# skokec/DAU-ConvNet

Measured on AMD Instinct MI355X. Metric: DAU fwd+bwd GSamples/s (N*H*W/s), higher is better.
Workload: dtype f32

## Files before the change

### dau-convnet_amd/csrc/dau_conv_api.hip

```cpp
#include <cmath>
#include <cstdarg>
#include <cstdio>
#include <algorithm>
#include <atomic>
#include <cstring>
#include <memory>
#include <mutex>
#include <new>
#include <string>
#include <utility>
#include <vector>

#include "dau_common.hpp"
#include "dau_tiled.hpp"

using namespace dau;

namespace {

thread_local std::string g_last_error;

int fail(int code, const char* fmt, ...) {
    char buf[512];
    va_list ap;
// ... 641 lines not shown
    if (!plan || !info) return fail(DAU_INVALID_ARGUMENT, "null argument");
    info->offset_bucket = plan->bucket;
    info->blur_support = plan->blur_k;
    info->algo_forward = plan->algo_fwd;
    info->algo_backward = plan->algo_bwd;
    info->drop_last_col = plan->drop_col;
    info->drop_last_row = plan->drop_row;
    const BucketSet& top = plan->top();
    const bool* s0 = plan->sets[0].has;
    const bool tiled_fwd = plan->algo_fwd == DAU_ALGO_TILED;
    info->gather_patch = tiled_fwd ? top.tiled[kFwd].tiles_x * top.tiled[kFwd].tile_w : 0;
    info->gather_stack = tiled_fwd ? top.tiled[kFwd].stack : 0;
    info->dot_windows = plan->algo_bwd == DAU_ALGO_TILED ? top.tiled_dot.windows : 0;
    info->gather_windows = tiled_fwd ? top.tiled[kFwd].windows : 0;
    info->bucket_sets = plan->dynamic ? plan->nsets : 1;
    const bool dense_reachable = s0[kBf16R4] && (plan->nsets == 1 || plan->dynamic);
    info->gather_dense_bf16 = dense_reachable ? (s0[kWgradR4] ? 2 : 1) : 0;
    info->batch_slab_gather = top.slab_gather;
    info->batch_slab_dot = top.slab_dot;
    info->dot_region = top.has[kTiledDot] ? top.tiled_dot.region_cols * 100 + top.tiled_dot.region_rows : 0;
    info->gather_fblock = tiled_fwd ? top.tiled[kFwd].fblock : 0;
    info->gather_variant = tiled_fwd ? top.tiled[kFwd].variant : -1;
    info->dense_bf16_radius3 = dense_reachable && plan->dynamic && s0[kBf16R3] ? (s0[kWgradR3] ? 2 : 1) : 0;
    info->gather_dense_split = 0;
    if (plan->dynamic && tiled_fwd)
        for (int m = kSplit2; m <= kSplit4; ++m)
            if (s0[m]) info->gather_dense_split |= 1 << kRadius[m];
    if (plan->sets[0].ring) info->gather_dense_split |= 1 << 5;
    if (plan->dynamic && tiled_fwd && s0[kLine4]) info->gather_dense_split |= 1 << 6;
    if (plan->dynamic && tiled_fwd && s0[kLine8]) info->gather_dense_split |= 1 << 7;
    return DAU_OK;
}

int dau_conv_workspace_bytes(const dau_conv_plan* plan, int pass, size_t* bytes_out) {
    if (!plan || !bytes_out) return fail(DAU_INVALID_ARGUMENT, "null argument");
    if (pass == DAU_PASS_FORWARD) *bytes_out = carve_forward(plan, nullptr).bytes;
    else if (pass == DAU_PASS_BACKWARD) *bytes_out = carve_backward(plan, nullptr).bytes;
    else if (pass == DAU_PASS_EPILOGUE_BACKWARD)
        *bytes_out = epilogue_grad_workspace_bytes(plan->sh.N, plan->sh.F, plan->sh.H, plan->sh.W, plan->act(), plan->d.flags & DAU_FLAG_IO_NHWC);
    else return fail(DAU_INVALID_ARGUMENT, "pass must be DAU_PASS_FORWARD, DAU_PASS_BACKWARD or DAU_PASS_EPILOGUE_BACKWARD");
    return DAU_OK;
}

namespace {
int forward_pass(const dau_conv_plan* p, void* stream, const float* x, const float* w, const float* mu1,
                 const float* mu2, const float* sigma, float* y, void* workspace, size_t workspace_bytes, const Epilogue& epi) {
    if (!p || !x || !w || !mu1 || !mu2 || !sigma || !y || !workspace) return fail(DAU_INVALID_ARGUMENT, "null argument");
    FwdWs ws = carve_forward(p, workspace);
    if (workspace_bytes < ws.bytes)
        return fail(DAU_INVALID_ARGUMENT, "workspace too small: %zu < %zu", workspace_bytes, ws.bytes);
    hipStream_t st = static_cast<hipStream_t>(stream);
    if (int rc = ensure_attrs(p)) return rc;
    DAU_HIP(hipMemsetAsync(ws.status, 0, sizeof(Status), st));
    launch_synth_filters(st, sigma, p->blur_k, p->d.flags, ws.filters);
    launch_prepare_units(st, w, mu1, mu2, p->sh, p->d.number_units_ignore, p->d.flags, p->bucket, false, ws.table, ws.status,
                         p->host_status, -1, p->sets[0].has[kLine4] ? ws.status : nullptr);
    run_gather_sum(p, st, kFwd, x, y, ws.filters, ws.table, ws.status, ws.gather, epi);
    DAU_HIP(hipPeekAtLastError());
    return DAU_OK;
}
}

int dau_conv_forward(const dau_conv_plan* p, void* stream, const float* x, const float* w, const float* mu1,
                     const float* mu2, const float* sigma, float* y, void* workspace, size_t workspace_bytes) {
    return forward_pass(p, stream, x, w, mu1, mu2, sigma, y, workspace, workspace_bytes, Epilogue{});
}
// ... 248 lines not shown
```

### dau-convnet_amd/csrc/dau_tiled.hpp

```cpp
#pragma once
#include "dau_common.hpp"

namespace dau {

struct TiledConfig {
    int N, Cin, Cout, G, H, W;
    int R;
    int blur_k;
    int NP;
    int windows;
    int stack;
    int patches;
    int rows, pitch;
    int tiles_x, tiles_y;
    int tile_w;
    int fblock;
    int variant;
    int debug;
    int act;
    int nhwc;
    int in_relu;
};

bool tiled_gather_configure(int N, int Cin, int Cout, int G, int H, int W, int R, int blur_k, int act, TiledConfig* cfg);
// ... 82 lines not shown
    int debug;
    int nhwc;
    int in_relu;
};

bool tiled_dot_configure(const Shape& sh, int R, int blur_k, int act, int ignore, TiledDotConfig* cfg);
size_t tiled_dot_workspace_bytes(const TiledDotConfig& cfg);
void tiled_dot_prepare(hipStream_t st, const TiledDotConfig& cfg, const float* x, const float* dy,
                       const float* filters, const UnitRef* table_bare, int drop_col, int drop_row, void* workspace,
                       const Guard& guard);
void tiled_dot_run(hipStream_t st, const TiledDotConfig& cfg, float* r4, void* workspace, const Guard& guard, bool accumulate);
void tiled_dot_init(const TiledDotConfig& cfg);

void launch_blur4_pack(hipStream_t st, const float* x, const float* filters, int N, int C, int cstride, int H, int W, int Hp,
                       int Wp, int blur_k, int act, float* xk, const Guard& guard, unsigned* kmax = nullptr, bool nhwc = false,
                       bool in_relu = false);
void blur4_pack_init(int blur_k, bool kmax = false, bool nhwc = false);
bool blur4_pack_fits(int blur_k, int Hp, int Wp);

void launch_dot_reduce(hipStream_t st, const void* partial, int partial_f32, long n, int G, int F, int g_split, int slabs0,
                       int slabs1, int zero_from, bool accumulate, float* r4, const Guard& guard);

struct SplitDotConfig {
    Shape sh;
    int blur_k;
    int RW;
    int act;
    int e_limbs;
    int nhwc;
    int in_relu;
};
bool split_dot_configure(const Shape& sh, int blur_k, int act, SplitDotConfig* cfg);
size_t split_dot_workspace_bytes(const SplitDotConfig& cfg);
void split_dot_init(const SplitDotConfig& cfg);
void split_dot_prepare(hipStream_t st, const SplitDotConfig& cfg, const float* x, const float* dy, const float* filters,
                       int drop_col, int drop_row, void* workspace, const Guard& guard);
void split_dot_run(hipStream_t st, const SplitDotConfig& cfg, const UnitRef* table, float* r4, void* workspace, const Guard& guard);

struct WgradConfig {
    Shape sh;
    int blur_k;
    int SB, FB, NC;
    int HsT, WsT, WT, nseg;
    int splits;
    int Hp, Wp;
    bool fused;
};
#define DAU_DECLARE_DENSE_WGRAD(NS)                                                                                            \
    namespace NS {                                                                                                            \
    bool dense_wgrad_configure(const Shape& sh, int blur_k, bool bf16, WgradConfig* cfg);                                     \
    size_t dense_wgrad_workspace_bytes(const WgradConfig& cfg);                                                               \
    void dense_wgrad_init(const WgradConfig& cfg);                                                                            \
    void dense_wgrad_run(hipStream_t st, const WgradConfig& cfg, const float* x, const float* dy, const float* filters,       \
                         const UnitRef* table, int drop_col, int drop_row, float* r4, void* workspace, const Guard& guard, int nk); \
    }
DAU_DECLARE_DENSE_WGRAD(r4)
DAU_DECLARE_DENSE_WGRAD(r3)

size_t epilogue_grad_workspace_bytes(long N, int F, int H, int W, int act, bool nhwc);
bool epilogue_grad_run(hipStream_t st, long N, int F, int H, int W, int act, bool nhwc, const float* dy, const float* y, bool relu,
                       float* dz, float* dbias, void* workspace);

}
```

### dau-convnet_amd/csrc/k_split_dot.hip

```cpp
#include <algorithm>
#include <cfloat>

#include "dau_tiled.hpp"

namespace dau {

typedef _Float16 h8 __attribute__((ext_vector_type(8)));
typedef float f4s __attribute__((ext_vector_type(4)));

namespace {

constexpr int kSdWaves = 8;
constexpr int kSdAS = 2;
constexpr int kSdGT = 4;
constexpr int kSdSB = kSdWaves * kSdAS;
constexpr int kSdFB = 16;
constexpr int kSdR = 4;
constexpr int kSdRH = 4;
constexpr int kSdFlushItems = 16;
constexpr unsigned kVmcnt0 = 0x0F70, kVmcnt8 = 0x0F78;

inline size_t rup(size_t v, size_t a = 256) { return (v + a - 1) / a * a; }

struct SdGeom {
    int Hq, Wq, rq, cq, XTr, XTc, EYs, EXs, octs, nfb, nsb, ngb, items, chunks, per, NP;
};

SdGeom sd_geom(const SplitDotConfig& c) {
    const Shape& s = c.sh;
    SdGeom g{};
    g.Hq = (s.H + 1 + kSdRH - 1) / kSdRH * kSdRH;
    g.Wq = (s.W + 1 + c.RW - 1) / c.RW * c.RW;
    g.rq = g.Hq / kSdRH; g.cq = g.Wq / c.RW;
    g.XTr = g.Hq + 1; g.XTc = g.Wq + 1;
    g.EYs = g.Hq + 2 * kSdR; g.EXs = g.Wq + 2 * kSdR;
    g.octs = (s.N + 7) / 8;
    g.NP = (s.N + 1) / 2;
    g.nfb = (s.F + kSdFB - 1) / kSdFB;
    g.nsb = (s.S + kSdSB - 1) / kSdSB;
    g.ngb = (s.G + kSdGT - 1) / kSdGT;
    g.items = g.octs * g.rq * g.cq;
    const int per_chunk = g.nfb * g.nsb * g.ngb;
    int chunks = (1024 + per_chunk - 1) / per_chunk;
    chunks = std::max(1, std::min(chunks, g.items));
    g.per = (g.items + chunks - 1) / chunks;
    g.chunks = (g.items + g.per - 1) / g.per;
    return g;
}

struct SdLayout { size_t maxes_off, xk_off, xs_off, es_off, partial_off, total; };

SdLayout sd_layout(const SplitDotConfig& c, const SdGeom& g) {
    const Shape& s = c.sh;
    SdLayout l{};
    size_t off = 0;
    l.maxes_off = off; off += rup((size_t)(s.S * kNumK + s.F) * 4);
    l.xk_off = off; off += rup((size_t)g.NP * s.S * s.H * s.W * 32);
    l.xs_off = off; off += rup((size_t)g.octs * s.S * kNumK * g.XTr * g.XTc * 32 + 32);
    l.es_off = off; off += rup((size_t)g.octs * g.nfb * g.EYs * g.EXs * 256 * c.e_limbs);
    l.partial_off = off; off += rup((size_t)g.chunks * kNumK * s.S * s.G * s.F * 4);
    l.total = off;
    return l;
}

__device__ __forceinline__ int sd_shift(unsigned maxbits) {
    if (maxbits == 0u) return 0;
// ... 533 lines not shown
        const float sc = f < F ? ldexpf(1.0f, sd_shift(emax[f])) : 0.0f;
        float v[8];
#pragma unroll
        for (int n = 0; n < 8; ++n) {
            const int img = oct * 8 + n;
            const bool ok = in && img < N;
            v[n] = mask_act(load_act(dy, ok ? nhwc_index(img, f, y, x, F, H, W) : 0, act), ok);
        }
        h8 hi, lo;
#pragma unroll
        for (int n = 0; n < 8; ++n) {
            if constexpr (LIMBS == 2) {
                _Float16 h, l;
                split_limbs(v[n] * sc, &h, &l);
                hi[n] = h; lo[n] = l;
            } else {
                hi[n] = (_Float16)(v[n] * sc);
            }
        }
        dst[lx * (kSdFB * LIMBS) + fl] = hi;
        if constexpr (LIMBS == 2) dst[lx * (kSdFB * LIMBS) + kSdFB + fl] = lo;
    }
}

struct SdArgs {
    const h8* xs;
    const char* es;
    const unsigned* xmax;
    const unsigned* emax;
    const UnitRef* table;
    float* partial;
    int S, F, G;
    int nfb, nsb, ngb, per, items, rq, cq, XTr, XTc, EYs, EXs;
    Guard guard;
};

__device__ __forceinline__ void sd_glds16(const char* src, unsigned dst) {
    unsigned keep;
    asm volatile("s_mov_b32 %0, m0\n\ts_mov_b32 m0, %2\n\ts_nop 0\n\tglobal_load_lds_dwordx4 %1, off\n\ts_mov_b32 m0, %0"
                 : "=&s"(keep) : "v"(src), "s"(dst) : "memory");
}

#ifndef DAU_SD_STEP_LOADS
__device__ __forceinline__ h8 sd_next_col(h8 cur, h8 nxt, int dx) {
    typedef int i4s __attribute__((ext_vector_type(4)));
    const i4s c = __builtin_bit_cast(i4s, cur), n = __builtin_bit_cast(i4s, nxt);
    i4s r;
#pragma unroll
    for (int d = 0; d < 4; ++d)
        r[d] = __builtin_amdgcn_update_dpp(0, dx ? c[d] : n[d], 0xB1 , 0xF, 0xF, true);
    return __builtin_bit_cast(h8, r);
}
#endif

template <int RW, int EL>
__device__ __forceinline__ void sd_dot_body(const SdArgs& a) {
    extern __shared__ __attribute__((aligned(16))) char lds[];
    if (!guard_pass(a.guard)) return;
    constexpr int WL = RW + 2 * kSdR, WR = kSdRH + 2 * kSdR;
    constexpr int kRing = WR + kSdRH;
    constexpr int PB = EL * 256;
    constexpr unsigned RB = WL * PB;
    constexpr int kRowPieces = (RB + 1023) / 1024;
    static_assert((kRing & (kRing - 1)) == 0, "ring slot = (origin + row) & (kRing - 1)");
    static_assert(RW % 2 == 0, "A fragment sets by the parity of the K step / of the pair of K steps");
#ifdef DAU_SD_STEP_LOADS
// ... 13 lines not shown
    const int fl = lane & 15, j = lane >> 4;
    const int f = fb * kSdFB + fl;
    const bool f_ok = f < a.F;
    const unsigned lds0 = (unsigned)(uintptr_t)(__attribute__((address_space(3))) char*)lds;
    const int m = lane & 15, ak = m >> 2, ady = (m >> 1) & 1, adx = m & 1;
    const size_t xplane = (size_t)a.XTr * a.XTc;
    unsigned aoff[kSdAS];
    int sidx[kSdAS];
    bool s_ok[kSdAS];
    unsigned uw[kSdAS][kSdGT];
    f4s wb[kSdAS][kSdGT];
    float run[kSdAS][kSdGT];
#pragma unroll
    for (int i = 0; i < kSdAS; ++i) {
        const int s = sb * kSdSB + wave * kSdAS + i;
        s_ok[i] = s < a.S;
        sidx[i] = s_ok[i] ? s : a.S - 1;
        aoff[i] = (unsigned)((((size_t)sidx[i] * kNumK + ak) * xplane + (size_t)(j + ady) * a.XTc + adx) * 2);
#pragma unroll
        for (int gg = 0; gg < kSdGT; ++gg) {
            const int g = gb * kSdGT + gg;
            UnitRef u{0, 0, 0.0f, 0.0f, 0.0f, 0.0f};
            if (s_ok[i] && g < a.G && f_ok) u = a.table[((size_t)sidx[i] * a.G + g) * a.F + f];
            uw[i][gg] = (unsigned)(j - u.oy + kSdR) | (unsigned)((kSdR - u.ox) * PB + fl * 16) << 4;
            wb[i][gg] = f4s{u.w00, u.w01, u.w10, u.w11};
            run[i][gg] = 0.0f;
        }
    }
    int shx[kSdAS];
    const int she = f_ok ? sd_shift(a.emax[f]) : 0;
#pragma unroll
    for (int i = 0; i < kSdAS; ++i) shx[i] = sd_shift(a.xmax[sidx[i] * kNumK + j]);
    auto flush = [&]() {
#pragma unroll
        for (int i = 0; i < kSdAS; ++i) {
#pragma unroll
            for (int gg = 0; gg < kSdGT; ++gg) {
                const int g = gb * kSdGT + gg;
                if (s_ok[i] && g < a.G && f_ok) {
                    const float v = ldexpf(ldexpf(run[i][gg], -shx[i]), -she);
                    float* dst = a.partial + ((((size_t)chunk * kNumK + j) * a.S + sidx[i]) * a.G + g) * a.F + f;
                    __hip_atomic_fetch_add(dst, v, __ATOMIC_RELAXED, __HIP_MEMORY_SCOPE_AGENT);
                }
                run[i][gg] = 0.0f;
            }
        }
    };
    const int per_oct = a.rq * a.cq;
    auto item_off = [&](int item) {
        const int oct = item / per_oct, reg = item - oct * per_oct, rx = reg / a.rq, ry = reg - rx * a.rq;
        return ((size_t)oct * a.S * kNumK * xplane + (size_t)(ry * kSdRH) * a.XTc + (size_t)rx * RW) * 2;
    };
    auto fill = [&](int oct, int ry, int rx, int w0, int nrows, int origin) {
#ifndef DAU_SD_DIAG_NOFILL
        const char* src = a.es + ((((size_t)oct * a.nfb + fb) * a.EYs + (size_t)(ry * kSdRH + w0)) * a.EXs + (size_t)rx * RW) * PB;
        for (int u = wave_u; u < nrows * kRowPieces; u += kSdWaves) {
            const int rr = u / kRowPieces, pc = u - rr * kRowPieces;
            const unsigned within = pc * 1024 + lane * 16;
            const unsigned slot = (unsigned)(origin + w0 + rr) & (kRing - 1);
            if (within < RB) sd_glds16(src + (size_t)rr * a.EXs * PB + within, lds0 + slot * RB + pc * 1024);
        }
#endif
    };
    h8 ahi[2][kSdAS], alo[2][kSdAS];
    if (it0 < it1) {
#pragma unroll
        for (int p = 0; p < 2; ++p)
#pragma unroll
            for (int i = 0; i < kSdAS; ++i) {
                const h8* ap = a.xs + item_off(it0) + (size_t)p * kSdAStride + aoff[i];
                ahi[p][i] = ap[0]; alo[p][i] = ap[1];
            }
    }
    int since_flush = 0;
    int origin = 0;
    for (int it = it0; it < it1; ++it) {
        const int oct = it / per_oct, reg = it - oct * per_oct, rx = reg / a.rq, ry = reg - rx * a.rq;
        __builtin_amdgcn_s_waitcnt(kVmcnt8);
        __syncthreads();
        if (it > it0 && ry > 0) {
            origin = (origin + kSdRH) & (kRing - 1);
        } else {
            origin = 0;
            fill(oct, ry, rx, 0, WR, 0);
            __builtin_amdgcn_s_waitcnt(kVmcnt0);
            __syncthreads();
        }
        if (it + 1 < it1 && ry + 1 < a.rq) fill(oct, ry, rx, WR, kSdRH, origin);
        int base[kSdAS][kSdGT];
#pragma unroll
        for (int i = 0; i < kSdAS; ++i)
#pragma unroll
            for (int gg = 0; gg < kSdGT; ++gg)
                base[i][gg] = (int)((((unsigned)origin + (uw[i][gg] & 15u)) & (kRing - 1)) * RB + (uw[i][gg] >> 4));
#ifdef DAU_SD_DIAG_AFIXED
        const size_t ioff = item_off(it0), ioff_next = ioff;
#else
        const size_t ioff = item_off(it);
        const size_t ioff_next = item_off(it + 1 < it1 ? it + 1 : it);
#endif
        f4s part[kSdAS][kSdGT];
#pragma unroll
        for (int i = 0; i < kSdAS; ++i)
#pragma unroll
            for (int gg = 0; gg < kSdGT; ++gg) part[i][gg] = f4s{0.0f, 0.0f, 0.0f, 0.0f};
#ifdef DAU_SD_DIAG_NOA
#define SD_LOAD_A(P, i, an)
#else
#define SD_LOAD_A(P, i, an) { const h8* ap = a.xs + (an) + aoff[i]; ahi[P][i] = ap[0]; alo[P][i] = ap[1]; }
#endif
#define SD_READ_B(i, bh, bl)                                                                                    \
    _Pragma("unroll") for (int gg = 0; gg < kSdGT; ++gg) {                                                      \
        const char* bp = lds + base[i][gg] + k * PB;                                                            \
        bh[gg] = *reinterpret_cast<const h8*>(bp);                                                              \
        if constexpr (EL == 2) bl[gg] = *reinterpret_cast<const h8*>(bp + 256);                                 \
    }
#define SD_GROUP(i, AH, AL, bh, bl, AFTER)                                                                      \
    __builtin_amdgcn_sched_barrier(0);                                                                          \
    _Pragma("unroll") for (int gg = 0; gg < kSdGT; ++gg) {                                                      \
        part[i][gg] = __builtin_amdgcn_mfma_f32_16x16x32_f16(AH, bh[gg], part[i][gg], 0, 0, 0);                 \
        part[i][gg] = __builtin_amdgcn_mfma_f32_16x16x32_f16(AL, bh[gg], part[i][gg], 0, 0, 0);                 \
        if constexpr (EL == 2) part[i][gg] = __builtin_amdgcn_mfma_f32_16x16x32_f16(AH, bl[gg], part[i][gg], 0, 0, 0); \
    }                                                                                                           \
    AFTER                                                                                                       \
    __builtin_amdgcn_sched_barrier(0);
#define SD_STEP(kk, AH, AL, AFTER0, AFTER1)                                                                     \
    {                                                                                                           \
        const int k = (kk);                                                                                     \
        h8 b0h[kSdGT], b0l[kSdGT], b1h[kSdGT], b1l[kSdGT];                                                      \
        SD_READ_B(0, b0h, b0l)                                                                                  \
        SD_READ_B(1, b1h, b1l)                                                                                  \
        SD_GROUP(0, AH[0], AL[0], b0h, b0l, AFTER0)                                                             \
        SD_GROUP(1, AH[1], AL[1], b1h, b1l, AFTER1)                                                             \
    }
        static_assert(kSdAS == 2, "two groups per K step");
#ifdef DAU_SD_STEP_LOADS
#define SD_STEP1(P, kk)                                                                                         \
    {                                                                                                           \
        const size_t an = (kk) + 2 < RW ? ioff + (size_t)((kk) + 2) * 2 : ioff_next + (size_t)((kk) + 2 - RW) * 2; \
        (void)an;                                                                                               \
        SD_STEP(kk, ahi[P], alo[P], SD_LOAD_A(P, 0, an), SD_LOAD_A(P, 1, an))                                   \
    }
#pragma unroll 1
        for (int k2 = 0; k2 < RW; k2 += 2) {
            SD_STEP1(0, k2)
            SD_STEP1(1, k2 + 1)
        }
#undef SD_STEP1
#else
        h8 aqh[kSdAS], aql[kSdAS];
#define SD_NEXT_COL(P, i)                                                                                       \
    aqh[i] = sd_next_col(ahi[P][i], ahi[1 - (P)][i], adx);                                                      \
    aql[i] = sd_next_col(alo[P][i], alo[1 - (P)][i], adx);
#define SD_PAIR(P, rr)                                                                                          \
    {                                                                                                           \
        const size_t an = ioff + (size_t)((rr) + 2) * 4;                                                        \
        (void)an;                                                                                               \
        SD_STEP(2 * (rr), ahi[P], alo[P], SD_NEXT_COL(P, 0) SD_LOAD_A(P, 0, an), SD_NEXT_COL(P, 1) SD_LOAD_A(P, 1, an)) \
        SD_STEP(2 * (rr) + 1, aqh, aql, , )                                                                     \
    }
#define SD_PAIR_LAST(P, rr)                                                                                     \
    {                                                                                                           \
        SD_STEP(2 * (rr), ahi[P], alo[P], SD_NEXT_COL(P, 0) SD_LOAD_A(0, 0, ioff_next), SD_NEXT_COL(P, 1) SD_LOAD_A(0, 1, ioff_next)) \
        SD_STEP(2 * (rr) + 1, aqh, aql, SD_LOAD_A(1, 0, ioff_next + 4), SD_LOAD_A(1, 1, ioff_next + 4))         \
    }
        constexpr int kPairs = RW / 2, kLoopPairs = (kPairs - 1) / 2 * 2;
#pragma unroll 1
        for (int r2 = 0; r2 < kLoopPairs; r2 += 2) {
            SD_PAIR(0, r2)
            SD_PAIR(1, r2 + 1)
        }
        if constexpr (kPairs - kLoopPairs == 2) {
            SD_PAIR(0, kPairs - 2)
            SD_PAIR_LAST(1, kPairs - 1)
        } else {
            SD_PAIR_LAST(0, kPairs - 1)
        }
#undef SD_NEXT_COL
#undef SD_PAIR
#undef SD_PAIR_LAST
#endif
#undef SD_READ_B
#undef SD_GROUP
#undef SD_LOAD_A
#undef SD_STEP
#pragma unroll
        for (int i = 0; i < kSdAS; ++i)
#pragma unroll
            for (int gg = 0; gg < kSdGT; ++gg) {
                const int g = gb * kSdGT + gg;
                const bool ok = s_ok[i] && g < a.G && f_ok;
                const f4s p = part[i][gg], w = wb[i][gg];
                float v = w[0] * p[0];
                v = fmaf(w[1], p[1], v);
                v = fmaf(w[2], p[2], v);
                v = fmaf(w[3], p[3], v);
                run[i][gg] += ok ? v : 0.0f;
            }
        if (++since_flush == kSdFlushItems) { flush(); since_flush = 0; }
    }
    asm volatile("s_waitcnt vmcnt(0)" ::: "memory");
    if (since_flush) flush();
}

template <int RW>
__global__ void __launch_bounds__(kSdWaves * 64) __attribute__((amdgpu_waves_per_eu(2, 2))) split_gather_dot_kernel(const SdArgs a) {
    sd_dot_body<RW, 2>(a);
}

template <int RW>
__global__ void __launch_bounds__(kSdWaves * 64) __attribute__((amdgpu_waves_per_eu(2, 2))) sd_e1_dot_kernel(const SdArgs a) {
    sd_dot_body<RW, 1>(a);
}

template <int RW, int EL>
void launch_sd(hipStream_t st, const SdArgs* a, int grid) {
    auto kern = [] { if constexpr (EL == 2) return split_gather_dot_kernel<RW>; else return sd_e1_dot_kernel<RW>; }();
    const size_t lds = (size_t)(2 * kSdRH + 2 * kSdR) * (RW + 2 * kSdR) * 256 * EL;
    if (!a) { (void)hipFuncSetAttribute(reinterpret_cast<const void*>(kern), hipFuncAttributeMaxDynamicSharedMemorySize, 160 * 1024); return; }
    hipLaunchKernelGGL(kern, dim3(grid), dim3(kSdWaves * 64), lds, st, *a);
}
bool sd_walks(const SplitDotConfig& c) {
#if defined(DAU_SD_XK_COPY) || defined(DAU_SD_STAGE_REF)
    return false;
#else
    const SdGeom g = sd_geom(c);
    const long nct = (g.XTc + kXwCols - 1) / kXwCols;
    return !c.nhwc && (c.blur_k == 5 || c.blur_k == 7 || c.blur_k == 9) && (long)g.octs * c.sh.S * nct < (1L << 31);
#endif
}
template <int K, bool STORE>
void launch_xk_walk(hipStream_t st, const XkWalkArgs& a, int grid) {
// ... 19 lines not shown
        else launch_sd<12, 1>(st, a, grid);
    } else {
        if (RW == 10) launch_sd<10, 2>(st, a, grid);
        else launch_sd<12, 2>(st, a, grid);
    }
}

}

bool split_dot_configure(const Shape& sh, int blur_k, int act, SplitDotConfig* cfg) {
    int best = 0;
    long best_cost = 1L << 40;
    for (int rw = 12; rw >= 10; rw -= 2) {
        const long wq = (sh.W + 1 + rw - 1) / rw * rw;
        const long cost = wq * (rw + 2) * (60 / rw);
        if (cost < best_cost) { best_cost = cost; best = rw; }
    }
    if ((size_t)(2 * kSdRH + 2 * kSdR) * (best + 2 * kSdR) * 512 > 160 * 1024) return false;
    if (!blur4_pack_fits(blur_k, sh.H, sh.W)) return false;
    SplitDotConfig c{};
    c.sh = sh; c.blur_k = blur_k; c.RW = best; c.act = act;
#ifdef DAU_SD_BF16_E2
    c.e_limbs = 2;
#else
    c.e_limbs = act == kActBF16 ? 1 : 2;
#endif
    const SdGeom g = sd_geom(c);
    if ((long)g.EXs * 512 * 32 > (1L << 31)) return false;
    *cfg = c;
    return true;
}

size_t split_dot_workspace_bytes(const SplitDotConfig& c) { return sd_layout(c, sd_geom(c)).total; }

void split_dot_init(const SplitDotConfig& c) {
    dispatch_sd(c.RW, c.e_limbs, nullptr, nullptr, 0);
#ifndef DAU_SD_STAGE_REF
    blur4_pack_init(c.blur_k, true, c.nhwc != 0);
#else
    blur4_pack_init(c.blur_k, false, c.nhwc != 0);
#endif
}

void split_dot_prepare(hipStream_t st, const SplitDotConfig& c, const float* x, const float* dy, const float* filters,
                       int drop_col, int drop_row, void* workspace, const Guard& guard) {
    const SdGeom g = sd_geom(c);
    const SdLayout l = sd_layout(c, g);
    const Shape& s = c.sh;
    char* ws = static_cast<char*>(workspace);
    unsigned* xmax = reinterpret_cast<unsigned*>(ws + l.maxes_off);
    unsigned* emax = xmax + s.S * kNumK;
    float* xk = reinterpret_cast<float*>(ws + l.xk_off);
    (void)hipMemsetAsync(xmax, 0, (size_t)(s.S * kNumK + s.F) * 4, st);
    (void)hipMemsetAsync(ws + l.partial_off, 0, (size_t)g.chunks * kNumK * s.S * s.G * s.F * 4, st);
    const int HW = s.H * s.W;
    const bool walks = sd_walks(c);
    h8* xs = reinterpret_cast<h8*>(ws + l.xs_off);
#ifndef DAU_SD_STAGE_REF
    if (walks) dispatch_xk_walk<false>(st, c, g, x, filters, xmax, xs, guard);
    else launch_blur4_pack(st, x, filters, s.N, s.S, s.S, s.H, s.W, s.H, s.W, c.blur_k, c.act, xk, guard, xmax, c.nhwc != 0, c.in_relu != 0);
#else
    launch_blur4_pack(st, x, filters, s.N, s.S, s.S, s.H, s.W, s.H, s.W, c.blur_k, c.act, xk, guard, nullptr, c.nhwc != 0, c.in_relu != 0);
    const int xsplit = std::max(1, std::min(16, 2048 / std::max(1, s.S)));
    hipLaunchKernelGGL(sd_absmax_x_kernel, dim3(s.S * xsplit), dim3(256), 0, st, xk, g.NP, s.S, HW, xsplit, xmax, guard);
#endif
    if (c.nhwc) {
// ... 31 lines not shown
    w.nct = (g.EXs + kSeCols - 1) / kSeCols;
    w.wlim = drop_col ? s.W - 1 : s.W; w.hlim = drop_row ? s.H - 1 : s.H; w.act = c.act; w.guard = guard;
    const long cols = (long)g.octs * g.nfb * w.nct, nb = (5120 + cols - 1) / cols;
    const int rb = DAU_TUNE_INT("DAU_SD_STAGE_E_RB", 0);
    w.RB = rb > 0 ? rb : std::max(4, (int)((g.EYs + nb - 1) / nb));
    w.nbands = (g.EYs + w.RB - 1) / w.RB;
    hipLaunchKernelGGL(sd_stage_e_kernel, dim3((unsigned)(cols * w.nbands)), dim3(64), 0, st, w);
    return;
#else
    hipLaunchKernelGGL(sd_stage_e_kernel, dim3((unsigned)(g.octs * g.nfb * g.EYs * nct)), dim3(256), 0, st, dy, emax, s.N, s.F, s.H,
                       s.W, g.nfb, g.EYs, g.EXs, nct, tx, drop_col, drop_row, c.act, reinterpret_cast<h8*>(ws + l.es_off), guard);
#endif
#else
    hipLaunchKernelGGL(sd_stage_e_kernel, dim3(4096), dim3(256), 0, st, dy, emax, s.N, s.F, s.H, s.W, g.octs, g.nfb, g.EYs, g.EXs,
                       drop_col, drop_row, c.act, c.nhwc, reinterpret_cast<h8*>(ws + l.es_off), guard);
#endif
}

void split_dot_run(hipStream_t st, const SplitDotConfig& c, const UnitRef* table, float* r4, void* workspace, const Guard& guard) {
    const SdGeom g = sd_geom(c);
    const SdLayout l = sd_layout(c, g);
    const Shape& s = c.sh;
    char* ws = static_cast<char*>(workspace);
    SdArgs a{};
    a.xs = reinterpret_cast<const h8*>(ws + l.xs_off);
    a.es = ws + l.es_off;
    a.xmax = reinterpret_cast<const unsigned*>(ws + l.maxes_off);
    a.emax = a.xmax + s.S * kNumK;
    a.table = table;
    a.partial = reinterpret_cast<float*>(ws + l.partial_off);
    a.S = s.S; a.F = s.F; a.G = s.G;
    a.nfb = g.nfb; a.nsb = g.nsb; a.ngb = g.ngb; a.per = g.per; a.items = g.items; a.rq = g.rq; a.cq = g.cq;
    a.XTr = g.XTr; a.XTc = g.XTc; a.EYs = g.EYs; a.EXs = g.EXs;
    a.guard = guard;
    dispatch_sd(c.RW, c.e_limbs, st, &a, g.chunks * g.nfb * g.nsb * g.ngb);
    launch_dot_reduce(st, a.partial, 1, (long)kNumK * s.S * s.G * s.F, s.G, s.F, s.G, g.chunks, g.chunks, s.G, false, r4, guard);
}

}
```

### dau-convnet_amd/dau_conv/_capi.py

```python
import ctypes
import os

import torch

_HERE = os.path.dirname(os.path.abspath(__file__))
_LIB_PATH = os.environ.get("DAU_CONV_LIB") or os.path.join(_HERE, "libdau_conv_hip.so")

DAU_OK, DAU_INVALID_ARGUMENT, DAU_FAILED_PRECONDITION, DAU_INTERNAL = 0, 1, 2, 3

FLAG_USE_INTERPOLATION = 1 << 0
FLAG_UNIT_TESTING = 1 << 1
FLAG_SINGLE_DIM_KERNEL = 1 << 2
FLAG_FORBID_POSITIVE_DIM1 = 1 << 3
FLAG_IO_BF16 = 1 << 4
FLAG_STATIC_BUCKET = 1 << 5
FLAG_DENSE_BF16 = 1 << 6
FLAG_DENSE_WGRAD_NEVER = 1 << 7
FLAG_DENSE_WGRAD_ALWAYS = 1 << 8
FLAG_DENSE_SPLIT_F16 = 1 << 9
FLAG_NO_DENSE_SPLIT = 1 << 10
FLAG_DENSE_SPLIT_LINE = 1 << 15
FLAG_DENSE_SPLIT_OUTLIERS = 1 << 12
FLAG_IO_F16 = 1 << 11
FLAG_IO_NHWC = 1 << 13
# ... 30 lines not shown
        ("mu_learning_rate_factor", ctypes.c_float),
    ]


class _Info(ctypes.Structure):
    _fields_ = [(n, ctypes.c_int32) for n in
                ("offset_bucket", "blur_support", "algo_forward", "algo_backward", "drop_last_col", "drop_last_row",
                 "gather_patch", "gather_stack", "dot_windows", "gather_windows", "bucket_sets", "gather_dense_bf16", "batch_slab_gather", "batch_slab_dot", "dot_region", "gather_fblock", "gather_variant", "dense_bf16_radius3", "gather_dense_split")]


def _load():
    if not os.path.exists(_LIB_PATH):
        raise ImportError(
            "dau_conv: %s not found. Build it with `make -C dau-convnet_amd/csrc` (hipcc, gfx950) or "
            "`python -c 'import __graft_entry__ as g; g.build()'`. There is no CPU fallback." % _LIB_PATH)
    lib = ctypes.CDLL(_LIB_PATH)
    vp, fp, ip = ctypes.c_void_p, ctypes.c_void_p, ctypes.c_void_p
    lib.dau_conv_abi_version.restype = ctypes.c_int
    lib.dau_conv_last_error.restype = ctypes.c_char_p
    lib.dau_conv_build_id.restype = ctypes.c_char_p
    lib.dau_conv_plan_create.argtypes = [ctypes.POINTER(_Desc), ctypes.POINTER(vp)]
    lib.dau_conv_plan_destroy.argtypes = [vp]
    lib.dau_conv_plan_get_info.argtypes = [vp, ctypes.POINTER(_Info)]
    lib.dau_conv_workspace_bytes.argtypes = [vp, ctypes.c_int, ctypes.POINTER(ctypes.c_size_t)]
    lib.dau_conv_forward.argtypes = [vp, vp, fp, fp, fp, fp, fp, fp, vp, ctypes.c_size_t]
    lib.dau_conv_backward.argtypes = [vp, vp] + [fp] * 11 + [vp, ctypes.c_size_t, ctypes.c_int]
    lib.dau_conv_backward_param_sums.argtypes = [vp, vp] + [fp] * 6 + [vp, ctypes.c_size_t]
    lib.dau_conv_finalize_param_grads.argtypes = [vp, vp] + [fp] * 6 + [ctypes.c_int]
    lib.dau_conv_check_status.argtypes = [vp, vp, vp, ctypes.POINTER(ctypes.c_float)]
    if hasattr(lib, "dau_conv_gather_outlier_status"):
        lib.dau_conv_gather_outlier_status.argtypes = [vp, vp, vp, ctypes.POINTER(ctypes.c_int32), ctypes.POINTER(ctypes.c_int32)]
    if hasattr(lib, "dau_conv_gather_line_status"):
        lib.dau_conv_gather_line_status.argtypes = [vp, vp, vp, ctypes.POINTER(ctypes.c_int32), ctypes.POINTER(ctypes.c_int32)]
    if hasattr(lib, "dau_conv_forward_epilogue"):
        lib.dau_conv_epilogue_supported.argtypes = [vp, ctypes.c_int]
        lib.dau_conv_forward_epilogue.argtypes = [vp, vp, fp, fp, fp, fp, fp, fp, ctypes.c_int, fp, vp, ctypes.c_size_t]
        lib.dau_conv_epilogue_backward.argtypes = [vp, vp, fp, fp, ctypes.c_int, fp, fp, vp, ctypes.c_size_t]
    if hasattr(lib, "dau_conv_forward_residual"):
        lib.dau_conv_forward_residual.argtypes = [vp, vp, fp, fp, fp, fp, fp, fp, fp, ctypes.c_int, fp, vp, ctypes.c_size_t]
    lib.dau_conv_last_status.argtypes = [vp, ctypes.POINTER(ctypes.c_float), ctypes.POINTER(ctypes.c_int32)]
    lib.dau_conv_filters.argtypes = [vp, vp, fp, fp]
    lib.dau_conv_unit_table.argtypes = [vp, vp, fp, fp, fp, ctypes.c_int, vp]
    lib.dau_conv_filter_support.argtypes = [ctypes.c_float]
    lib.dau_conv_filter_support.restype = ctypes.c_int
    lib.dau_conv_profile_begin.argtypes = [vp]
    lib.dau_conv_profile_end.argtypes = [vp, ctypes.POINTER(ctypes.c_double), ctypes.POINTER(ctypes.c_int32)]
    if lib.dau_conv_abi_version() != 4:
        raise ImportError("dau_conv: ABI version mismatch in %s" % _LIB_PATH)
    return lib


lib = _load()


def filter_support(sigma):
    return int(lib.dau_conv_filter_support(ctypes.c_float(float(sigma))))


def build_id():
    return lib.dau_conv_build_id().decode()


def _check(code):
    if code == DAU_OK:
        return
    msg = lib.dau_conv_last_error().decode("utf-8", "replace")
# ... 184 lines not shown
                                                    _ptr(out), _ptr(ws), ws.numel()))
        self._last_ws = ws
        return out

    def finalize_param_grads(self, sums, w, need_mask=NEED_DW | NEED_DMU1 | NEED_DMU2 | NEED_DSIGMA):
        pshape = (1, self.S, self.G, self.F)
        _req(sums, "sums", (4, self.S, self.G, self.F))
        _req(w, "weights", pshape)
        dev = _same_device(sums, w)
        new = lambda: torch.empty(pshape, dtype=torch.float32, device=dev)
        with torch.cuda.device(dev):
            dw = new() if need_mask & NEED_DW else None
            dmu1 = new() if need_mask & NEED_DMU1 else None
            dmu2 = new() if need_mask & NEED_DMU2 else None
            dsigma = new() if need_mask & NEED_DSIGMA else None
            _check(lib.dau_conv_finalize_param_grads(self._h, _stream(dev), _ptr(sums), _ptr(w), _ptr(dw), _ptr(dmu1),
                                                     _ptr(dmu2), _ptr(dsigma), int(need_mask)))
        return dw, dmu1, dmu2, dsigma

    def check_status(self):
        mx = ctypes.c_float()
        dev = self._last_ws.device
        with torch.cuda.device(dev):
            _check(lib.dau_conv_check_status(self._h, _stream(dev), _ptr(self._last_ws), ctypes.byref(mx)))
        return mx.value

    def outlier_status(self):
        units, taken = ctypes.c_int32(), ctypes.c_int32()
        dev = self._last_ws.device
        with torch.cuda.device(dev):
            _check(lib.dau_conv_gather_outlier_status(self._h, _stream(dev), _ptr(self._last_ws), ctypes.byref(units), ctypes.byref(taken)))
        return units.value, bool(taken.value)

    def line_status(self):
        units, taken = ctypes.c_int32(), ctypes.c_int32()
        dev = self._last_ws.device
        with torch.cuda.device(dev):
            _check(lib.dau_conv_gather_line_status(self._h, _stream(dev), _ptr(self._last_ws), ctypes.byref(units), ctypes.byref(taken)))
        return units.value, taken.value

    def last_status(self):
        mx, valid = ctypes.c_float(), ctypes.c_int32()
        _check(lib.dau_conv_last_status(self._h, ctypes.byref(mx), ctypes.byref(valid)))
        return mx.value if valid.value else None

    def profile_begin(self):
        _check(lib.dau_conv_profile_begin(self._h))

    def profile_end(self):
        ms = (ctypes.c_double * 3)()
        n = (ctypes.c_int32 * 3)()
        _check(lib.dau_conv_profile_end(self._h, ms, n))
        return {name: (ms[i], n[i]) for i, name in enumerate(("gather_sum_fwd", "gather_sum_dx", "gather_dot"))}

    def filters(self, sigma):
        k = self.info["blur_support"]
        out = torch.empty((6, k, k), dtype=torch.float32, device=sigma.device)
        with torch.cuda.device(sigma.device):
            _check(lib.dau_conv_filters(self._h, _stream(sigma.device), _ptr(sigma), _ptr(out)))
        return out

    def unit_table(self, mu1, mu2, w=None, form=0):
        units = self.S * self.G * self.F
        raw = torch.empty((units, 6), dtype=torch.int32, device=mu1.device)
        with torch.cuda.device(mu1.device):
            _check(lib.dau_conv_unit_table(self._h, _stream(mu1.device), _ptr(w), _ptr(mu1), _ptr(mu2), int(form), _ptr(raw)))
# ... 2 lines not shown
```

### include/dau_conv.h

```cpp
#ifndef DAU_CONV_H_
#define DAU_CONV_H_

#include <stddef.h>
#include <stdint.h>

#ifdef __cplusplus
extern "C" {
#endif

#define DAU_CONV_ABI_VERSION 4

#if defined(__GNUC__)
#define DAU_API __attribute__((visibility("default")))
#else
#define DAU_API
#endif

enum {
    DAU_OK = 0,
    DAU_INVALID_ARGUMENT = 1,
    DAU_FAILED_PRECONDITION = 2,
    DAU_INTERNAL = 3
};

// ... 58 lines not shown

typedef struct dau_conv_plan_info {
    int32_t offset_bucket;
    int32_t blur_support;
    int32_t algo_forward;
    int32_t algo_backward;
    int32_t drop_last_col;
    int32_t drop_last_row;
    int32_t gather_patch;
    int32_t gather_stack;
    int32_t dot_windows;
    int32_t gather_windows;
    int32_t bucket_sets;
    int32_t gather_dense_bf16;
    int32_t batch_slab_gather;
    int32_t batch_slab_dot;
    int32_t dot_region;
    int32_t gather_fblock;
    int32_t gather_variant;
    int32_t dense_bf16_radius3;
    int32_t gather_dense_split;
} dau_conv_plan_info;

DAU_API int dau_conv_abi_version(void);
DAU_API const char *dau_conv_build_id(void);
DAU_API const char *dau_conv_last_error(void);

DAU_API int dau_conv_filter_support(float sigma);

DAU_API int dau_conv_plan_create(const dau_conv_desc *desc, dau_conv_plan **plan_out);
DAU_API int dau_conv_plan_destroy(dau_conv_plan *plan);
DAU_API int dau_conv_plan_get_info(const dau_conv_plan *plan, dau_conv_plan_info *info);
DAU_API int dau_conv_workspace_bytes(const dau_conv_plan *plan, int pass, size_t *bytes_out);

DAU_API int dau_conv_forward(const dau_conv_plan *plan, void *stream, const float *x, const float *w,
                     const float *mu1, const float *mu2, const float *sigma, float *y,
                     void *workspace, size_t workspace_bytes);

DAU_API int dau_conv_epilogue_supported(const dau_conv_plan *plan, int epilogue);
DAU_API int dau_conv_forward_epilogue(const dau_conv_plan *plan, void *stream, const float *x, const float *w,
                     const float *mu1, const float *mu2, const float *sigma, const float *bias, int epilogue,
                     float *y, void *workspace, size_t workspace_bytes);

DAU_API int dau_conv_forward_residual(const dau_conv_plan *plan, void *stream, const float *x, const float *w,
                     const float *mu1, const float *mu2, const float *sigma, const float *bias, const float *residual,
                     int epilogue, float *y, void *workspace, size_t workspace_bytes);

DAU_API int dau_conv_epilogue_backward(const dau_conv_plan *plan, void *stream, const float *dy, const float *y, int epilogue,
                     float *dz, float *dbias, void *workspace, size_t workspace_bytes);

DAU_API int dau_conv_backward(const dau_conv_plan *plan, void *stream, const float *x, const float *dy,
                      const float *w, const float *mu1, const float *mu2, const float *sigma,
                      float *dx, float *dw, float *dmu1, float *dmu2, float *dsigma,
                      void *workspace, size_t workspace_bytes, int need_mask);

DAU_API int dau_conv_backward_param_sums(const dau_conv_plan *plan, void *stream, const float *x, const float *dy,
                                 const float *mu1, const float *mu2, const float *sigma, float *sums_out,
                                 void *workspace, size_t workspace_bytes);
DAU_API int dau_conv_finalize_param_grads(const dau_conv_plan *plan, void *stream, const float *sums, const float *w,
                                  float *dw, float *dmu1, float *dmu2, float *dsigma, int need_mask);

DAU_API int dau_conv_check_status(const dau_conv_plan *plan, void *stream, const void *workspace,
                          float *max_abs_mu_out);

DAU_API int dau_conv_gather_outlier_status(const dau_conv_plan *plan, void *stream, const void *workspace,
                                   int32_t *outlier_units, int32_t *ring_taken);
// ... 19 lines not shown
```

Measured before the change: 0.01914.

## Add thin last-row item path to split-dot kernel to skip padded K steps

When the padded height leaves a single live row in the last region of a strip, the split-dot kernel now processes that item with a specialized 'thin' path. This path runs only three K fragments with adjusted A offsets and LDS base offsets instead of the full RW steps. The item loop is restructured into templated full, before-thin and thin variants. It also adds readfirstlane on the LDS destination and a geometry query API. The aim is to avoid MFMA work on padding rows, at the cost of more code paths, register pressure and risk around index adjustments.

```diff
diff --git a/dau-convnet_amd/csrc/dau_conv_api.hip b/dau-convnet_amd/csrc/dau_conv_api.hip
--- a/dau-convnet_amd/csrc/dau_conv_api.hip
+++ b/dau-convnet_amd/csrc/dau_conv_api.hip
@@ -697,6 +697,21 @@
     return DAU_OK;
 }
 
+int dau_conv_split_dot_geometry(const dau_conv_plan* plan, int32_t* region_width, int32_t* strip_items, int32_t* strip_k_steps) {
+    if (!plan) return fail(DAU_INVALID_ARGUMENT, "null argument");
+    int rw = 0, items = 0, steps = 0;
+    for (int i = 0; i < plan->nsets && !rw; ++i) {
+        const BucketSet& bs = plan->sets[i];
+        if (!bs.has[kSplitDot]) continue;
+        rw = bs.sdot.RW;
+        split_dot_strip(bs.sdot, &items, &steps);
+    }
+    if (region_width) *region_width = rw;
+    if (strip_items) *strip_items = items;
+    if (strip_k_steps) *strip_k_steps = steps;
+    return DAU_OK;
+}
+
 int dau_conv_workspace_bytes(const dau_conv_plan* plan, int pass, size_t* bytes_out) {
     if (!plan || !bytes_out) return fail(DAU_INVALID_ARGUMENT, "null argument");
     if (pass == DAU_PASS_FORWARD) *bytes_out = carve_forward(plan, nullptr).bytes;
diff --git a/dau-convnet_amd/csrc/dau_tiled.hpp b/dau-convnet_amd/csrc/dau_tiled.hpp
--- a/dau-convnet_amd/csrc/dau_tiled.hpp
+++ b/dau-convnet_amd/csrc/dau_tiled.hpp
@@ -138,6 +138,7 @@
 };
 bool split_dot_configure(const Shape& sh, int blur_k, int act, SplitDotConfig* cfg);
 size_t split_dot_workspace_bytes(const SplitDotConfig& cfg);
+void split_dot_strip(const SplitDotConfig& cfg, int* items, int* k_steps);
 void split_dot_init(const SplitDotConfig& cfg);
 void split_dot_prepare(hipStream_t st, const SplitDotConfig& cfg, const float* x, const float* dy, const float* filters,
                        int drop_col, int drop_row, void* workspace, const Guard& guard);
diff --git a/dau-convnet_amd/csrc/k_split_dot.hip b/dau-convnet_amd/csrc/k_split_dot.hip
--- a/dau-convnet_amd/csrc/k_split_dot.hip
+++ b/dau-convnet_amd/csrc/k_split_dot.hip
@@ -22,8 +22,16 @@
 
 inline size_t rup(size_t v, size_t a = 256) { return (v + a - 1) / a * a; }
 
+#ifdef DAU_SD_NO_THIN
+constexpr bool kSdThin = false;
+#else
+constexpr bool kSdThin = true;
+#endif
+
 struct SdGeom {
     int Hq, Wq, rq, cq, XTr, XTc, EYs, EXs, octs, nfb, nsb, ngb, items, chunks, per, NP;
+    int thin;
+    int strip_steps;
 };
 
 SdGeom sd_geom(const SplitDotConfig& c) {
@@ -32,6 +40,8 @@
     g.Hq = (s.H + 1 + kSdRH - 1) / kSdRH * kSdRH;
     g.Wq = (s.W + 1 + c.RW - 1) / c.RW * c.RW;
     g.rq = g.Hq / kSdRH; g.cq = g.Wq / c.RW;
+    g.thin = kSdThin && (s.H + 1) % kSdRH == 1 && g.rq >= 2;
+    g.strip_steps = (g.rq - g.thin) * c.RW + g.thin * ((c.RW + kSdRH - 1) / kSdRH);
     g.XTr = g.Hq + 1; g.XTc = g.Wq + 1;
     g.EYs = g.Hq + 2 * kSdR; g.EXs = g.Wq + 2 * kSdR;
     g.octs = (s.N + 7) / 8;
@@ -631,6 +641,7 @@
     float* partial;
     int S, F, G;
     int nfb, nsb, ngb, per, items, rq, cq, XTr, XTc, EYs, EXs;
+    int thin;
     Guard guard;
 };
 
@@ -710,6 +721,8 @@
 #pragma unroll
     for (int i = 0; i < kSdAS; ++i) shx[i] = sd_shift(a.xmax[sidx[i] * kNumK + j]);
     auto flush = [&]() {
+        int jf = j;
+        asm volatile("" : "+v"(jf));
 #pragma unroll
         for (int i = 0; i < kSdAS; ++i) {
 #pragma unroll
@@ -717,7 +730,7 @@
                 const int g = gb * kSdGT + gg;
                 if (s_ok[i] && g < a.G && f_ok) {
                     const float v = ldexpf(ldexpf(run[i][gg], -shx[i]), -she);
-                    float* dst = a.partial + ((((size_t)chunk * kNumK + j) * a.S + sidx[i]) * a.G + g) * a.F + f;
+                    float* dst = a.partial + ((((size_t)chunk * kNumK + jf) * a.S + sidx[i]) * a.G + g) * a.F + f;
                     __hip_atomic_fetch_add(dst, v, __ATOMIC_RELAXED, __HIP_MEMORY_SCOPE_AGENT);
                 }
                 run[i][gg] = 0.0f;
@@ -736,23 +749,37 @@
             const int rr = u / kRowPieces, pc = u - rr * kRowPieces;
             const unsigned within = pc * 1024 + lane * 16;
             const unsigned slot = (unsigned)(origin + w0 + rr) & (kRing - 1);
-            if (within < RB) sd_glds16(src + (size_t)rr * a.EXs * PB + within, lds0 + slot * RB + pc * 1024);
+            if (within < RB) sd_glds16(src + (size_t)rr * a.EXs * PB + within, __builtin_amdgcn_readfirstlane(lds0 + slot * RB + pc * 1024));
         }
 #endif
     };
+    auto thin_adjust = [&]() {
+        int jj = j;
+        asm volatile("" : "+v"(jj));
+        return (unsigned)(jj * 2) - (unsigned)(jj * a.XTc * 2);
+    };
+    constexpr int kThinStride = 2 * kSdRH;
+    constexpr int kThinSteps = (RW + kSdRH - 1) / kSdRH;
+    static_assert(kThinSteps == 3, "a thin item: sets 0 and 1, then the third fragment");
+    auto is_thin = [&](int item) { return a.thin && item % a.rq == a.rq - 1; };
     h8 ahi[2][kSdAS], alo[2][kSdAS];
     if (it0 < it1) {
+        const bool th = is_thin(it0);
+        const unsigned adj0 = th ? thin_adjust() : 0u;
+        const size_t stride0 = th ? kThinStride : kSdAStride;
 #pragma unroll
         for (int p = 0; p < 2; ++p)
 #pragma unroll
             for (int i = 0; i < kSdAS; ++i) {
-                const h8* ap = a.xs + item_off(it0) + (size_t)p * kSdAStride + aoff[i];
+                const h8* ap = a.xs + item_off(it0) + (size_t)p * stride0 + (aoff[i] + adj0);
                 ahi[p][i] = ap[0]; alo[p][i] = ap[1];
             }
     }
     int since_flush = 0;
     int origin = 0;
-    for (int it = it0; it < it1; ++it) {
+    constexpr int kItemFull = 0, kItemBeforeThin = 1, kItemThin = 2;
+    auto item = [&](const int it, auto kind_c) {
+        constexpr bool thin = decltype(kind_c)::value == kItemThin, next_thin = decltype(kind_c)::value == kItemBeforeThin;
         const int oct = it / per_oct, reg = it - oct * per_oct, rx = reg / a.rq, ry = reg - rx * a.rq;
         __builtin_amdgcn_s_waitcnt(kVmcnt8);
         __syncthreads();
@@ -765,28 +792,36 @@
             __syncthreads();
         }
         if (it + 1 < it1 && ry + 1 < a.rq) fill(oct, ry, rx, WR, kSdRH, origin);
+        const unsigned jt = thin ? (unsigned)j : 0u;
         int base[kSdAS][kSdGT];
 #pragma unroll
         for (int i = 0; i < kSdAS; ++i)
 #pragma unroll
             for (int gg = 0; gg < kSdGT; ++gg)
-                base[i][gg] = (int)((((unsigned)origin + (uw[i][gg] & 15u)) & (kRing - 1)) * RB + (uw[i][gg] >> 4));
+                base[i][gg] = (int)((((unsigned)origin + (uw[i][gg] & 15u) - jt) & (kRing - 1)) * RB + (uw[i][gg] >> 4) + jt * PB);
 #ifdef DAU_SD_DIAG_AFIXED
         const size_t ioff = item_off(it0), ioff_next = ioff;
 #else
         const size_t ioff = item_off(it);
         const size_t ioff_next = item_off(it + 1 < it1 ? it + 1 : it);
 #endif
+        unsigned nadj = 0u, tadj = 0u;
+        if constexpr (next_thin) nadj = thin_adjust();
+        if constexpr (thin) tadj = thin_adjust();
+        constexpr size_t nstep = next_thin ? kThinStride : kSdAStride;
+        (void)nadj; (void)tadj;
         f4s part[kSdAS][kSdGT];
 #pragma unroll
         for (int i = 0; i < kSdAS; ++i)
 #pragma unroll
             for (int gg = 0; gg < kSdGT; ++gg) part[i][gg] = f4s{0.0f, 0.0f, 0.0f, 0.0f};
 #ifdef DAU_SD_DIAG_NOA
-#define SD_LOAD_A(P, i, an)
+#define SD_LOAD_INTO(AH, AL, i, an, ladj)
 #else
-#define SD_LOAD_A(P, i, an) { const h8* ap = a.xs + (an) + aoff[i]; ahi[P][i] = ap[0]; alo[P][i] = ap[1]; }
-#endif
+#define SD_LOAD_INTO(AH, AL, i, an, ladj) { const h8* ap = a.xs + (an) + (aoff[i] + (ladj)); AH[i] = ap[0]; AL[i] = ap[1]; }
+#endif
+#define SD_LOAD_A(P, i, an) SD_LOAD_INTO(ahi[P], alo[P], i, an, 0u)
+#define SD_LOAD_NEXT(P, i, an) SD_LOAD_INTO(ahi[P], alo[P], i, an, nadj)
 #define SD_READ_B(i, bh, bl)                                                                                    \
     _Pragma("unroll") for (int gg = 0; gg < kSdGT; ++gg) {                                                      \
         const char* bp = lds + base[i][gg] + k * PB;                                                            \
@@ -811,13 +846,65 @@
         SD_GROUP(0, AH[0], AL[0], b0h, b0l, AFTER0)                                                             \
         SD_GROUP(1, AH[1], AL[1], b1h, b1l, AFTER1)                                                             \
     }
+        auto combine = [&]() {
+#pragma unroll
+            for (int i = 0; i < kSdAS; ++i)
+#pragma unroll
+                for (int gg = 0; gg < kSdGT; ++gg) {
+                    const int g = gb * kSdGT + gg;
+                    const bool ok = s_ok[i] && g < a.G && f_ok;
+                    const f4s p = part[i][gg], w = wb[i][gg];
+                    float v = w[0] * p[0];
+                    v = fmaf(w[1], p[1], v);
+                    v = fmaf(w[2], p[2], v);
+                    v = fmaf(w[3], p[3], v);
+                    run[i][gg] += ok ? v : 0.0f;
+                }
+        };
         static_assert(kSdAS == 2, "two groups per K step");
+        h8 aqh[kSdAS], aql[kSdAS];
+        if constexpr (thin) {
+#define SD_READ_BT(kk, i, bh, bl)                                                                                 \
+    _Pragma("unroll") for (int gg = 0; gg < kSdGT; ++gg) {                                                      \
+        const char* bp = lds + base[i][gg] + 4 * (kk) * PB - dead;                                               \
+        bh[gg] = *reinterpret_cast<const h8*>(bp);                                                              \
+        if constexpr (EL == 2) bl[gg] = *reinterpret_cast<const h8*>(bp + 256);                                 \
+    }
+#define SD_THIN_STEP(kk, AH, AL, AFTER0, AFTER1)                                                                \
+    {                                                                                                           \
+        const int dead = 4 * (kk) + kSdRH <= RW || 4 * (kk) + j < RW ? 0 : j * PB;                              \
+        h8 bh[kSdGT], bl[kSdGT];                                                                                \
+        SD_READ_BT(kk, 0, bh, bl)                                                                               \
+        SD_GROUP(0, AH[0], AL[0], bh, bl, AFTER0)                                                               \
+        SD_READ_BT(kk, 1, bh, bl)                                                                               \
+        SD_GROUP(1, AH[1], AL[1], bh, bl, AFTER1)                                                               \
+    }
+#define SD_LOAD_THIRD(i) SD_LOAD_INTO(aqh, aql, i, ioff + (size_t)(2 * kThinStride), tadj)
+            SD_THIN_STEP(0, ahi[0], alo[0], SD_LOAD_THIRD(0) SD_LOAD_THIRD(1) SD_LOAD_NEXT(0, 0, ioff_next), SD_LOAD_NEXT(0, 1, ioff_next))
+            SD_THIN_STEP(1, ahi[1], alo[1], SD_LOAD_NEXT(1, 0, ioff_next + nstep), SD_LOAD_NEXT(1, 1, ioff_next + nstep))
+            if constexpr (4 * kThinSteps > RW) {
+                const bool live = 4 * (kThinSteps - 1) + j < RW;
+                const h8 zero = {0, 0, 0, 0, 0, 0, 0, 0};
+#pragma unroll
+                for (int i = 0; i < kSdAS; ++i) { aqh[i] = live ? aqh[i] : zero; aql[i] = live ? aql[i] : zero; }
+            }
+            SD_THIN_STEP(2, aqh, aql, , )
+            combine();
+#pragma unroll
+            for (int p = 0; p < 2; ++p)
+#pragma unroll
+                for (int i = 0; i < kSdAS; ++i) asm volatile("" : "+v"(ahi[p][i]), "+v"(alo[p][i]));
+#undef SD_LOAD_THIRD
+#undef SD_THIN_STEP
+#undef SD_READ_BT
+        } else {
 #ifdef DAU_SD_STEP_LOADS
 #define SD_STEP1(P, kk)                                                                                         \
     {                                                                                                           \
-        const size_t an = (kk) + 2 < RW ? ioff + (size_t)((kk) + 2) * 2 : ioff_next + (size_t)((kk) + 2 - RW) * 2; \
-        (void)an;                                                                                               \
-        SD_STEP(kk, ahi[P], alo[P], SD_LOAD_A(P, 0, an), SD_LOAD_A(P, 1, an))                                   \
+        const size_t an = (kk) + 2 < RW ? ioff + (size_t)((kk) + 2) * 2 : ioff_next + (size_t)((kk) + 2 - RW) * nstep; \
+        const unsigned la = (kk) + 2 < RW ? 0u : nadj;                                                          \
+        (void)an; (void)la;                                                                                     \
+        SD_STEP(kk, ahi[P], alo[P], SD_LOAD_INTO(ahi[P], alo[P], 0, an, la), SD_LOAD_INTO(ahi[P], alo[P], 1, an, la)) \
     }
 #pragma unroll 1
         for (int k2 = 0; k2 < RW; k2 += 2) {
@@ -826,7 +913,6 @@
         }
 #undef SD_STEP1
 #else
-        h8 aqh[kSdAS], aql[kSdAS];
 #define SD_NEXT_COL(P, i)                                                                                       \
     aqh[i] = sd_next_col(ahi[P][i], ahi[1 - (P)][i], adx);                                                      \
     aql[i] = sd_next_col(alo[P][i], alo[1 - (P)][i], adx);
@@ -839,8 +925,8 @@
     }
 #define SD_PAIR_LAST(P, rr)                                                                                     \
     {                                                                                                           \
-        SD_STEP(2 * (rr), ahi[P], alo[P], SD_NEXT_COL(P, 0) SD_LOAD_A(0, 0, ioff_next), SD_NEXT_COL(P, 1) SD_LOAD_A(0, 1, ioff_next)) \
-        SD_STEP(2 * (rr) + 1, aqh, aql, SD_LOAD_A(1, 0, ioff_next + 4), SD_LOAD_A(1, 1, ioff_next + 4))         \
+        SD_STEP(2 * (rr), ahi[P], alo[P], SD_NEXT_COL(P, 0) SD_LOAD_NEXT(0, 0, ioff_next), SD_NEXT_COL(P, 1) SD_LOAD_NEXT(0, 1, ioff_next)) \
+        SD_STEP(2 * (rr) + 1, aqh, aql, SD_LOAD_NEXT(1, 0, ioff_next + nstep), SD_LOAD_NEXT(1, 1, ioff_next + nstep)) \
     }
         constexpr int kPairs = RW / 2, kLoopPairs = (kPairs - 1) / 2 * 2;
 #pragma unroll 1
@@ -858,24 +944,23 @@
 #undef SD_PAIR
 #undef SD_PAIR_LAST
 #endif
+            combine();
+        }
+#undef SD_LOAD_NEXT
+#undef SD_LOAD_INTO
 #undef SD_READ_B
 #undef SD_GROUP
 #undef SD_LOAD_A
 #undef SD_STEP
-#pragma unroll
-        for (int i = 0; i < kSdAS; ++i)
-#pragma unroll
-            for (int gg = 0; gg < kSdGT; ++gg) {
-                const int g = gb * kSdGT + gg;
-                const bool ok = s_ok[i] && g < a.G && f_ok;
-                const f4s p = part[i][gg], w = wb[i][gg];
-                float v = w[0] * p[0];
-                v = fmaf(w[1], p[1], v);
-                v = fmaf(w[2], p[2], v);
-                v = fmaf(w[3], p[3], v);
-                run[i][gg] += ok ? v : 0.0f;
-            }
         if (++since_flush == kSdFlushItems) { flush(); since_flush = 0; }
+    };
+    for (int it = it0; it < it1;) {
+        const int run_end = a.thin ? min(it1, it + (a.rq - 1 - it % a.rq)) : it1;
+        const int full_end = run_end < it1 ? run_end - 1 : run_end;
+#pragma unroll 1
+        for (; it < full_end; ++it) item(it, std::integral_constant<int, kItemFull>{});
+        if (it < run_end) { item(it, std::integral_constant<int, kItemBeforeThin>{}); ++it; }
+        if (it < it1) { item(it, std::integral_constant<int, kItemThin>{}); ++it; }
     }
     asm volatile("s_waitcnt vmcnt(0)" ::: "memory");
     if (since_flush) flush();
@@ -961,6 +1046,11 @@
 }
 
 size_t split_dot_workspace_bytes(const SplitDotConfig& c) { return sd_layout(c, sd_geom(c)).total; }
+
+void split_dot_strip(const SplitDotConfig& c, int* items, int* k_steps) {
+    const SdGeom g = sd_geom(c);
+    *items = g.rq; *k_steps = g.strip_steps;
+}
 
 void split_dot_init(const SplitDotConfig& c) {
     dispatch_sd(c.RW, c.e_limbs, nullptr, nullptr, 0);
@@ -1058,6 +1148,7 @@
     a.S = s.S; a.F = s.F; a.G = s.G;
     a.nfb = g.nfb; a.nsb = g.nsb; a.ngb = g.ngb; a.per = g.per; a.items = g.items; a.rq = g.rq; a.cq = g.cq;
     a.XTr = g.XTr; a.XTc = g.XTc; a.EYs = g.EYs; a.EXs = g.EXs;
+    a.thin = g.thin;
     a.guard = guard;
     dispatch_sd(c.RW, c.e_limbs, st, &a, g.chunks * g.nfb * g.nsb * g.ngb);
     launch_dot_reduce(st, a.partial, 1, (long)kNumK * s.S * s.G * s.F, s.G, s.F, s.G, g.chunks, g.chunks, s.G, false, r4, guard);
diff --git a/dau-convnet_amd/dau_conv/_capi.py b/dau-convnet_amd/dau_conv/_capi.py
--- a/dau-convnet_amd/dau_conv/_capi.py
+++ b/dau-convnet_amd/dau_conv/_capi.py
@@ -86,6 +86,8 @@
         lib.dau_conv_gather_outlier_status.argtypes = [vp, vp, vp, ctypes.POINTER(ctypes.c_int32), ctypes.POINTER(ctypes.c_int32)]
     if hasattr(lib, "dau_conv_gather_line_status"):
         lib.dau_conv_gather_line_status.argtypes = [vp, vp, vp, ctypes.POINTER(ctypes.c_int32), ctypes.POINTER(ctypes.c_int32)]
+    if hasattr(lib, "dau_conv_split_dot_geometry"):
+        lib.dau_conv_split_dot_geometry.argtypes = [vp] + [ctypes.POINTER(ctypes.c_int32)] * 3
     if hasattr(lib, "dau_conv_forward_epilogue"):
         lib.dau_conv_epilogue_supported.argtypes = [vp, ctypes.c_int]
         lib.dau_conv_forward_epilogue.argtypes = [vp, vp, fp, fp, fp, fp, fp, fp, ctypes.c_int, fp, vp, ctypes.c_size_t]
@@ -336,6 +338,11 @@
             _check(lib.dau_conv_gather_outlier_status(self._h, _stream(dev), _ptr(self._last_ws), ctypes.byref(units), ctypes.byref(taken)))
         return units.value, bool(taken.value)
 
+    def split_dot_geometry(self):
+        v = [ctypes.c_int32() for _ in range(3)]
+        _check(lib.dau_conv_split_dot_geometry(self._h, *[ctypes.byref(c) for c in v]))
+        return tuple(c.value for c in v)
+
     def line_status(self):
         units, taken = ctypes.c_int32(), ctypes.c_int32()
         dev = self._last_ws.device
diff --git a/include/dau_conv.h b/include/dau_conv.h
--- a/include/dau_conv.h
+++ b/include/dau_conv.h
@@ -114,6 +114,7 @@
 DAU_API int dau_conv_plan_destroy(dau_conv_plan *plan);
 DAU_API int dau_conv_plan_get_info(const dau_conv_plan *plan, dau_conv_plan_info *info);
 DAU_API int dau_conv_workspace_bytes(const dau_conv_plan *plan, int pass, size_t *bytes_out);
+DAU_API int dau_conv_split_dot_geometry(const dau_conv_plan *plan, int32_t *region_width, int32_t *strip_items, int32_t *strip_k_steps);
 
 DAU_API int dau_conv_forward(const dau_conv_plan *plan, void *stream, const float *x, const float *w,
                      const float *mu1, const float *mu2, const float *sigma, float *y,
```

Result: faster. 0.01937, median of 6 (+1.2%).
